# remis-thoughts/native-hdfs-fuse

Measured on AMD Instinct MI355X. Metric: GiB/s CRC32C, device-resident 64 KiB packets × 512 B chunks, 1/2/4/8 GPU, higher is better.
Workload: dtype u32

## Files before the change

### include/hdfs_crc32c_debug.h

```cpp
#ifndef HDFS_CRC32C_DEBUG_H
#define HDFS_CRC32C_DEBUG_H

#include <stddef.h>
#include <stdint.h>

#include "hdfs_crc32c.h"

#ifdef __cplusplus
extern "C" {
#endif


int crc32c_debug_plan(const crc32c_packet *pkts, size_t npkts, void *tiles, size_t tiles_cap, void *gen,
                      size_t gen_cap, uint64_t *ntiles, uint64_t *ngen);
int crc32c_debug_plan_abs(const crc32c_packet *pkts, size_t npkts, int absolute, void *tiles, size_t tiles_cap,
                          void *gen, size_t gen_cap, uint64_t *ntiles, uint64_t *ngen);

int crc32c_debug_write_plan(const crc32c_buffer *buffers, uint32_t n_buffers, uint64_t bufferoffset, uint64_t len,
                            uint64_t blockoffset, uint32_t packetsize, uint32_t bpc, uint64_t counts[6]);

size_t crc32c_debug_lds_image(void *dst, size_t cap, uint32_t *c_lg5, uint32_t *c_small4);

size_t crc32c_debug_lds_image_s4(void *dst, size_t cap, uint32_t flags);
void crc32c_debug_affine_constants(uint32_t flags, uint32_t *c_lg5, uint32_t *c_small4);

int crc32c_debug_blocks_fail_flushes(crc32c_blocks *q, uint32_t n);

int crc32c_debug_blocks_resident_inject(crc32c_blocks *q, int hold, uint32_t fail_waits);

int crc32c_debug_blocks_worker_cpu_ns(crc32c_blocks *q, uint64_t *ns);

uint64_t crc32c_debug_plan_block(const crc32c_plan *plan);

typedef struct crc32c_debug_build {
    uint32_t threads, waves_per_simd, mode, units_per_tile, grid;
} crc32c_debug_build;

int crc32c_debug_select_build(uint32_t ntiles, uint32_t ngen, uint32_t nseg, uint32_t nconst, uint32_t general,
// ... 44 lines not shown
```

### native-hdfs-fuse_amd/__init__.py

```python
from __future__ import annotations

import ctypes
import errno
import numbers
import os
import subprocess

import numpy as np

HERE = os.path.dirname(os.path.abspath(__file__))
LIB_PATH = os.path.join(HERE, "libhdfs_crc32c.so")
DEBUG_LIB_PATH = os.path.join(HERE, "libhdfs_crc32c_debug.so")
INCLUDE_DIR = os.path.join(os.path.dirname(HERE), "include")

CRC32C_BIG_ENDIAN = 0x1
CRC32C_TYPE_CRC32 = 0x2
CRC32C_DEVICE_ADDRESSES = 0x4
CRC32C_CPU_FALLBACK = 0x8
CRC32C_MULTI_SELF_SEND = 0x10
CRC32C_COUNT_COMPLETION = 0x20
CRC32C_MULTI_PIPELINE = 0x40
CRC32C_MULTI_PER_GROUP_RECV = 0x80
CRC32C_VERIFY_OVERLAP = 0x80000000
PATH_NONE, PATH_GPU, PATH_CPU = 0, 1, 2
# ... 165 lines not shown
        "crc32c_plan_exec": (i32, [vp, vp, vp, vp]),
        "crc32c_plan_destroy": (i32, [vp]),
        "crc32c_plan_nchecksums": (u64, [vp]),
        "crc32c_plan_payload_bytes": (u64, [vp]),
        "crc32c_chunks_dev": (i32, [vp, vp, sz, vp, vp, u32, vp]),
        "crc32c_batch_host": (i32, [vp, vp, vp, sz, vp, u32]),
        "crc32c_chunks": (i32, [vp, sz, u32, vp, u32]),
        "crc32c_multi_create": (i32, [vp, i32, pp]),
        "crc32c_multi_destroy": (i32, [vp]),
        "crc32c_multi_batch_host": (i32, [vp, vp, vp, sz, u32, vp, u32]),
        "crc32c_last_error": (ctypes.c_char_p, []),
        "crc32c_debug_plan": (i32, [vp, sz, vp, sz, vp, sz, ctypes.POINTER(u64), ctypes.POINTER(u64)]),
        "crc32c_debug_plan_abs": (i32, [vp, sz, i32, vp, sz, vp, sz, ctypes.POINTER(u64), ctypes.POINTER(u64)]),
        "crc32c_debug_lds_image": (sz, [vp, sz, vp, vp]),
        "crc32c_debug_lds_image_s4": (sz, [vp, sz, u32]),
        "crc32c_plan_verify": (i32, [vp, vp, vp, vp, vp]),
        "crc32c_plan_verify_bitmap": (i32, [vp, vp, vp, vp, vp, vp]),
        "crc32c_frame_packets": (sz, [vp, sz, vp, u32, u64, ctypes.c_int64, u32, vp, sz, vp]),
        "crc32c_block_md5": (None, [vp, sz, u32, vp]),
        "crc32c_md5_nblocks": (u64, [u64, u32]),
        "crc32c_md5_blocks": (i32, [vp, vp, u64, u32, u32, vp, vp]),
        "crc32c_md5_block_list": (i32, [vp, vp, vp, sz, u32, vp, vp]),
        "crc32c_plan_exec_blocks_md5": (i32, [vp, vp, vp, sz, vp, vp]),
        "crc32c_file_md5": (None, [vp, sz, vp]),
        "crc32c_combine": (u32, [u32, u32, u64, u32]),
        "crc32c_block_composite": (i32, [vp, sz, u32, u32, u32, vp]),
        "crc32c_file_composite": (i32, [vp, vp, sz, u32, vp]),
        "crc32c_composite_cells": (i32, [vp, vp, u64, u32, u32, u32, u32, vp, vp]),
        "crc32c_composite_block_list": (i32, [vp, vp, vp, vp, sz, u32, u32, vp, vp]),
        "crc32c_plan_exec_blocks_composite": (i32, [vp, vp, vp, sz, vp, vp]),
# ... 675 lines not shown
    n = int(lib().crc32c_debug_lds_image(None, 0, None, None))
    img = np.zeros(n, np.uint8)
    c_lg = np.zeros(5, np.uint32)
    c_small = np.zeros(4, np.uint32)
    lib().crc32c_debug_lds_image(_np_ptr(img), n, _np_ptr(c_lg), _np_ptr(c_small))
    return img, c_lg, c_small


def debug_lds_image_s4(flags: int = 0):
    n = int(lib().crc32c_debug_lds_image_s4(None, 0, flags))
    img = np.zeros(n, np.uint8)
    lib().crc32c_debug_lds_image_s4(_np_ptr(img), n, flags)
    return img


def debug_affine_constants(flags: int = 0):
    c_lg = np.zeros(5, np.uint32)
    c_small = np.zeros(4, np.uint32)
    lib().crc32c_debug_affine_constants(flags, _np_ptr(c_lg), _np_ptr(c_small))
    return c_lg, c_small
```

### native-hdfs-fuse_amd/csrc/crc32c_device.h

```cpp
#pragma once
#include <hip/hip_runtime.h>
#include <stdint.h>

#include "kernel_abi.h"

namespace hdfs_crc_dev {

using hdfs_crc::ConstRun;
using hdfs_crc::FastTile;
using hdfs_crc::GenItem;
using hdfs_crc::GenPiece;
using hdfs_crc::KParams;
using hdfs_crc::SegItem;
using hdfs_crc::kGeneralTile;
using hdfs_crc::kEpochWord;

constexpr uint32_t kLdsBytes = hdfs_crc::kKernelLdsBytes;
constexpr uint32_t kShiftOff = hdfs_crc::kKernelShiftOff;
constexpr uint32_t kStageBytes = (kLdsBytes + 1023u) / 1024u * 1024u;
static_assert(kStageBytes <= hdfs_crc::kTableAlloc, "staging reads past the device table");
constexpr uint32_t kS4Bytes = uint32_t(hdfs_crc::kS4Bytes);
constexpr uint32_t kS4NibOff = uint32_t(hdfs_crc::kS4NibOff);
constexpr uint32_t kS4ShiftOff = uint32_t(hdfs_crc::kS4ShiftOff);
constexpr uint32_t kS4StageBytes = (kS4Bytes + 1023u) / 1024u * 1024u;
// ... 56 lines not shown
    }
    return acc;
}

__device__ __forceinline__ uint32_t and_or(uint32_t a, uint32_t mask, uint32_t c) {
    uint32_t r;
    asm("v_and_or_b32 %0, %1, %2, %3" : "=v"(r) : "v"(a), "s"(mask), "v"(c));
    return r;
}

struct LaneCols {
    uint32_t col4;
    uint32_t hi;
    uint32_t nib;
    uint32_t toff;
};

constexpr int kImgFull = 0, kImgCompact = 2;
constexpr uint32_t kS4CNibOff = uint32_t(hdfs_crc::kS4CNibOff);
constexpr uint32_t kS4CShiftOff = uint32_t(hdfs_crc::kS4CShiftOff);
constexpr uint32_t kS4CStageBytes = (uint32_t(hdfs_crc::kS4CBytes) + 1023u) / 1024u * 1024u;

template <int IMG>
__device__ __forceinline__ LaneCols lane_cols(uint32_t q) {
    if (IMG == kImgCompact)
        return LaneCols{0u, 2048u, (q << 2) | kS4CNibOff, 1024u};
    return LaneCols{q << 2, (q << 2) | 65536u, (q << 2) | kS4NibOff, 128u};
}

template <int J>
__device__ __forceinline__ uint32_t byte_addr(uint32_t v, uint32_t base) {
    return __builtin_amdgcn_perm(v, base, 0x0C020000u | uint32_t(4 + J) << 8);
}

template <int IMG>
__device__ __forceinline__ uint32_t s4(const uint8_t *lds, const LaneCols &c, uint32_t v, uint32_t next) {
    if (IMG == kImgCompact) {
        const uint32_t a3 = lds_u32(lds, (__builtin_amdgcn_ubfe(v, 0, 8) << 2) + c.hi + c.toff);
        const uint32_t a2 = lds_u32(lds, (__builtin_amdgcn_ubfe(v, 8, 8) << 2) + c.hi);
        const uint32_t a1 = lds_u32(lds, (__builtin_amdgcn_ubfe(v, 16, 8) << 2) + c.toff);
        const uint32_t a0 = lds_u32(lds, (v >> 24) << 2);
        return xor3(xor3(a3, a2, a1), a0, next);
    }
    const uint32_t a3 = lds_u32(lds, byte_addr<0>(v, c.hi) + c.toff);
    const uint32_t a2 = lds_u32(lds, byte_addr<1>(v, c.hi));
    const uint32_t a1 = lds_u32(lds, byte_addr<2>(v, c.col4) + c.toff);
    const uint32_t a0 = lds_u32(lds, byte_addr<3>(v, c.col4));
    return xor3(xor3(a3, a2, a1), a0, next);
}

template <int DIAG, int IMG>
__device__ __forceinline__ uint32_t piece_lin_s4(const uint8_t *lds, uint4 d, const LaneCols &c) {
    if (DIAG == 1) return d.x ^ d.y ^ d.z ^ d.w;
    const uint32_t u = s4<IMG>(lds, c, s4<IMG>(lds, c, s4<IMG>(lds, c, d.x, d.y), d.z), d.w);
    const uint32_t xs[8] = {u << 8, u << 4, u, u >> 4, u >> 8, u >> 12, u >> 16, u >> 20};
    uint32_t r[8];
#pragma unroll
    for (int t = 0; t < 8; ++t) r[t] = lds_u32(lds, and_or(xs[t], 0x0F00u, c.nib) + (t >> 1) * 4096u + (t & 1) * 128u);
    return xor3(xor3(r[0], r[1], r[2]), xor3(r[3], r[4], r[5]), r[6] ^ r[7]);
}

template <bool S4, int DIAG, int IMG>
__device__ __forceinline__ uint32_t piece(const uint8_t *lds, uint4 d, const LaneCols &c) {
    if (S4) return piece_lin_s4<DIAG, IMG>(lds, d, c);
    return piece_lin<DIAG>(lds, d, c.col4);
}

template <bool S4, int IMG>
__device__ __forceinline__ uint32_t zshift(const uint8_t *lds, uint32_t s, uint32_t x) {
    const uint32_t base = (!S4 ? kShiftOff : IMG == kImgCompact ? kS4CShiftOff : kS4ShiftOff) + (s - 1u) * 512u;
    uint32_t r = 0;
#pragma unroll
    for (int t = 0; t < 8; ++t) r ^= lds_u32(lds, base + t * 64u + ((x >> (4 * t)) & 15u) * 4u);
    return r;
}

template <int CTRL>
__device__ __forceinline__ uint32_t dpp(uint32_t v) {
    return static_cast<uint32_t>(__builtin_amdgcn_update_dpp(0, static_cast<int>(v), CTRL, 0xF, 0xF, false));
}
constexpr int kDppXor1 = 0xB1;
constexpr int kDppXor2 = 0x4E;
constexpr int kDppXor8 = 0x128;

template <int XORMASK>
// ... 580 lines not shown

#include "crc32c_items.h"

template <int THREADS, int WPS, int MODE>
__global__ __launch_bounds__(THREADS, WPS) void hdfs_crc32c_plan_kernel(hdfs_crc::KParams p) {
    using namespace hdfs_crc_dev;
    constexpr bool NT = (MODE & kModeNt) != 0;
    constexpr bool S4 = (MODE & kModeS4) != 0;
    constexpr bool STAMPS = (MODE & kModeStamps) != 0;
    constexpr bool COMPDIAG = (MODE & kModeCompDiag) != 0;
    constexpr int DIAG = ((MODE & kModeMemDiag) ? 1 : 0) | ((MODE & kModeGDiagNoGather) ? 2 : 0) |
                         ((MODE & kModeGDiagNoMask) ? 4 : 0);
    constexpr bool NOSTAGE = (MODE & kModeNoStage) != 0;
    constexpr bool VERIFY = (MODE & kModeVerify) != 0;
    constexpr bool C = S4 && (MODE & kModeS4C) != 0;
    constexpr int IMG = C ? kImgCompact : kImgFull;
    constexpr bool GENERAL = (MODE & kModeGeneral) != 0;
    constexpr int GEN = !GENERAL ? 0
                                 : ((MODE & kModeNoGItems) ? 0 : kGenItems) |
                                       ((MODE & kModeNoShift) ? ((MODE & kModeGGroup2) ? kGenGroup2 : kGenGroup4)
                                                              : (kGenShift | kGenGroup2)) |
                                       ((MODE & kModeGHoist) ? kGenHoist : 0) | ((MODE & kModeHalfT) ? kGenHalf : 0) |
                                       ((!(MODE & (kModeNoGItems | kModeNoPadT))) ? kGenPadded : 0);
    constexpr bool EARLY = (MODE & kModeEarly) != 0;
    constexpr bool OVL = !EARLY && (MODE & kModeOvl) != 0;
    constexpr bool QUARTER = (MODE & kModeQuarter) != 0;
    constexpr bool XCDMAP = (MODE & kModeXcdMap) != 0;
    constexpr int SPLIT = (MODE & kModeHalves) ? 2 : 4;
    constexpr int AUX = NT ? 2 : 0;
    constexpr uint32_t kWaves = THREADS / 64;
    constexpr uint32_t kStage = !S4 ? kStageBytes : C ? kS4CStageBytes : kS4StageBytes;
    __shared__ __attribute__((aligned(16))) uint8_t lds[kStage + 32 + (VERIFY ? 4 * kBadList : 0)];
    uint32_t *pool_ctr = reinterpret_cast<uint32_t *>(lds + kStage);
    uint32_t *vacc = pool_ctr + 1;
    uint32_t *exit_ctr = pool_ctr + 5;
    const uint8_t *table = !S4 ? p.table : C ? p.table_s4 + hdfs_crc::kS4COff : p.table_s4;
    const int lane = int(threadIdx.x & 63u);
    const uint32_t wv = __builtin_amdgcn_readfirstlane(threadIdx.x >> 6);

    uint64_t t_start = 0, t_staged = 0;
    if (STAMPS) t_start = __builtin_amdgcn_s_memrealtime();

    const uint64_t nunits = QUARTER ? uint64_t(SPLIT) * p.ntiles : uint64_t(p.ntiles);
    const uint32_t rng = XCDMAP && (gridDim.x % 8u) == 0 ? (blockIdx.x % 8u) * (gridDim.x / 8u) + blockIdx.x / 8u
                                                         : blockIdx.x;
    const uint32_t tbeg = uint32_t((nunits * rng) / gridDim.x);
    const uint32_t tend = uint32_t((nunits * (rng + 1)) / gridDim.x);
    if (threadIdx.x == 0) {
        *pool_ctr = tbeg + kWaves;
        *exit_ctr = 0;
        if (VERIFY) {
// ... 7 lines not shown
    FastTile ft{0, 0, 0};
    uint4 v[9];
    uint32_t ev = 0;
    int kind = 1;
    auto load_next = [&](uint32_t j) {
        if (QUARTER) {
            kind = load_unit<AUX, COMPDIAG, VERIFY, GEN, SPLIT>(p, j, lane, ft, v, ev);
        } else {
            ft = tile_at(p, j);
            load_any<AUX, COMPDIAG, VERIFY, GEN>(p, ft, lane, v, ev);
        }
    };
    if (EARLY && t < tend) load_next(t);
    const bool tables = (p.ntiles | p.ngen | p.nseg) != 0;
    constexpr uint32_t kStageChunks = kStage / 1024u;
    constexpr uint32_t kNoZChunks = !S4 ? kStageChunks : C ? uint32_t(hdfs_crc::kS4CShiftOff / 1024u)
                                                           : uint32_t(hdfs_crc::kS4ShiftOff / 1024u);
    static_assert(!S4 || kNoZChunks * 1024u == (C ? hdfs_crc::kS4CShiftOff : hdfs_crc::kS4ShiftOff),
                  "the Z section starts on a staging chunk");
    const uint32_t nstage = p.skip_z ? kNoZChunks : kStageChunks;
    if (!NOSTAGE && tables) {
        const uint32_t rot = (blockIdx.x * 37u) % nstage;
        for (uint32_t i = wv; i < nstage; i += kWaves) {
            const uint32_t c = i + rot < nstage ? i + rot : i + rot - nstage;
            __builtin_amdgcn_global_load_lds(
                (const __attribute__((address_space(1))) void *)(table + c * 1024u + 16u * uint32_t(lane)),
                (__attribute__((address_space(3))) void *)(lds + c * 1024u), 16, 0, 0);
        }
    }
    if (OVL && t < tend) load_next(t);
    __syncthreads();
    if (STAMPS) t_staged = __builtin_amdgcn_s_memrealtime();
    if (VERIFY && blockIdx.x == 0 && wv == kWaves - 1) verify_init(p, lane);

// ... 55 lines not shown
```

### native-hdfs-fuse_amd/csrc/crc32c_runtime.hip

```cpp
#include <hip/hip_runtime.h>

#include <algorithm>
#include <atomic>
#include <cerrno>
#include <chrono>
#include <cstdarg>
#include <cstdio>
#include <cstdlib>
#include <cstring>
#include <memory>
#include <mutex>
#include <string>
#include <thread>
#include <vector>

#include "crc_math.h"
#include "hdfs_crc32c.h"
#include "hdfs_crc32c_debug.h"
#include "kernel_abi.h"
#include "plan.h"
#include "host_copy.h"
#include "runtime_internal.h"

namespace {
// ... 832 lines not shown
    HIP_TRY(preload_md5_kernels());
    HIP_TRY(preload_composite_kernels());
    c->host_pool.pinned = true;
    HIP_TRY(hipStreamCreateWithFlags(&c->upload_stream, hipStreamNonBlocking));
    for (int ty = 0; ty < 2; ++ty) {
        const uint32_t poly = ty ? kPolyIeee : kPoly;
        std::vector<uint8_t> img(kTableAlloc, 0);
        build_lds_image(img.data(), poly);
        affine_constants(c->c_lg[ty], c->c_small[ty], poly);
        HIP_TRY(hipMalloc(reinterpret_cast<void **>(&c->d_table[ty]), kTableAlloc));
        HIP_TRY(hipMemcpy(c->d_table[ty], img.data(), kTableAlloc, hipMemcpyHostToDevice));
        std::vector<uint8_t> img4(kTableAllocS4Full, 0);
        build_lds_image_s4(img4.data(), poly);
        compact_s4_image(img4.data(), img4.data() + kS4COff);
        zero_crc_table(reinterpret_cast<uint32_t *>(img4.data() + kZeroCrcOff), poly);
        HIP_TRY(hipMalloc(reinterpret_cast<void **>(&c->d_table_s4[ty]), kTableAllocS4Full));
        HIP_TRY(hipMemcpy(c->d_table_s4[ty], img4.data(), kTableAllocS4Full, hipMemcpyHostToDevice));
    }
    *out = c.release();
    return 0;
}

}

namespace {

void ctx_teardown(crc32c_ctx *ctx) {
    {
        DeviceGuard guard(ctx->device);
        for (Stage &s : ctx->stage) free_stage(s);
// ... 360 lines not shown
```

### native-hdfs-fuse_amd/csrc/crc_math.cpp

```cpp
#include "crc_math.h"

#include <cstring>
#include <mutex>
#include <vector>

namespace hdfs_crc {

namespace {
struct PolyTable {
    uint32_t t[256];
    std::once_flag once;
};
PolyTable g_tab[2];

void init_t0(uint32_t poly, uint32_t *t) {
    for (uint32_t b = 0; b < 256; ++b) {
        uint32_t r = b;
        for (int i = 0; i < 8; ++i) r = (r >> 1) ^ (poly & (0u - (r & 1u)));
        t[b] = r;
    }
}
}

const uint32_t *byte_table(uint32_t poly) {
// ... 131 lines not shown
                    zq.apply(s4_step(n << (4 * t), poly)));
    }
    std::vector<uint8_t> nib(kLdsBytes);
    build_lds_image(nib.data(), poly);
    std::memcpy(dst + kS4ShiftOff, nib.data() + kLdsShiftOff, kMaxShift * 512);
}

void compact_s4_image(const uint8_t *full, uint8_t *dst) {
    std::memset(dst, 0, kS4CBytes);
    for (uint32_t m = 0; m < 4; ++m)
        for (uint32_t b = 0; b < 256; ++b)
            std::memcpy(dst + m * 1024u + 4u * b, full + (m >> 1) * 65536u + b * 256u + (m & 1u) * 128u, 4);
    std::memcpy(dst + kS4CNibOff, full + kS4NibOff, kS4Bytes - kS4NibOff);
}

void affine_constants(uint32_t c_lg[5], uint32_t c_small[4], uint32_t poly) {
    for (int lg = 0; lg < 5; ++lg) c_lg[lg] = op_zeros(512ull << lg, poly).apply(0xffffffffu) ^ 0xffffffffu;
    for (int r = 0; r < 4; ++r) c_small[r] = op_zeros(r, poly).apply(0xffffffffu) ^ 0xffffffffu;
}

void zero_crc_table(uint32_t *dst, uint32_t poly) {
    uint32_t reg = 0xffffffffu;
    for (uint32_t n = 0; n <= kZeroCrcMax; ++n) {
        dst[n] = reg ^ 0xffffffffu;
        reg = append_zero_byte(reg, poly);
    }
}

}
```

### native-hdfs-fuse_amd/csrc/crc_math.h

```cpp
#pragma once
#include <cstddef>
#include <cstdint>

namespace hdfs_crc {

constexpr uint32_t kPoly = 0x82f63b78u;
constexpr uint32_t kPolyIeee = 0xedb88320u;

struct Gf2Op {
    uint32_t col[32];
    uint32_t apply(uint32_t v) const {
        uint32_t r = 0;
        for (int j = 0; v; ++j, v >>= 1)
            if (v & 1u) r ^= col[j];
        return r;
    }
};

const uint32_t *byte_table(uint32_t poly = kPoly);
uint32_t append_zero_byte(uint32_t reg, uint32_t poly = kPoly);
Gf2Op op_identity();
Gf2Op op_compose(const Gf2Op &a, const Gf2Op &b);
Gf2Op op_zeros(uint64_t nbytes, uint32_t poly = kPoly);
uint32_t shift_zeros(uint32_t reg, uint64_t nbytes, uint32_t poly = kPoly);
// ... 12 lines not shown
constexpr size_t kLdsShiftOff = 65536;
constexpr int kMaxShift = 15;
constexpr size_t kLdsBytes = kLdsPosBytes + kMaxShift * 512;

void build_lds_image(uint8_t *dst, uint32_t poly = kPoly);

constexpr size_t kS4NibOff = 131072;
constexpr size_t kS4ShiftOff = 147456;
constexpr size_t kS4Bytes = kS4ShiftOff + kMaxShift * 512;

constexpr size_t kS4CNibOff = 4096;
constexpr size_t kS4CShiftOff = kS4CNibOff + (kS4ShiftOff - kS4NibOff);
constexpr size_t kS4CBytes = kS4CShiftOff + kMaxShift * 512;
void compact_s4_image(const uint8_t *full, uint8_t *dst);

void build_lds_image_s4(uint8_t *dst, uint32_t poly = kPoly);
uint32_t s4_step(uint32_t u, uint32_t poly = kPoly);

void affine_constants(uint32_t c_lg[5], uint32_t c_small[4], uint32_t poly = kPoly);

constexpr uint32_t kZeroCrcMax = 8192;
void zero_crc_table(uint32_t *dst, uint32_t poly = kPoly);

}
```

### native-hdfs-fuse_amd/csrc/debug/crc32c_variants.hip

```cpp
#include "../crc32c_device.h"
#include "../runtime_internal.h"
#include "hdfs_crc32c_debug.h"

namespace {

using namespace hdfs_crc_dev;
constexpr int kS4Nt = kModeS4 | kModeNt | kModeGeneral;

struct Variant {
    int id;
    const char *name;
    uint32_t threads, wg_per_cu;
    bool exact;
    bool prod_grid = false;
};

constexpr Variant kVariants[] = {
    {0, "s4_nt", 768, 1, true},
    {1, "nibble_wg1024x2_nt", 1024, 2, true},
    {2, "s4_wg1024x1_nt", 1024, 1, true},
    {3, "s4_wg768x1_nt_memonly", 768, 1, false},
    {4, "s4_wg768x1_nt_compute_only", 768, 1, false},
    {5, "s4_wg768x1_nt_stamps", 768, 1, true},
    {6, "s4_wg768x1_nt_memonly_stamps", 768, 1, false},
// ... 33 lines not shown
    {82, "s4c_nt_quarter_nopad_prodgrid", 768, 1, true, true},
    {83, "s4c_nt_quarter_nopad_early_prodgrid", 768, 1, true, true},
    {84, "s4c_nt_nopad_prodgrid", 768, 1, true, true},
    {85, "s4c_nt_nopad_early_prodgrid", 768, 1, true, true},
    {86, "s4c_nt_halves_nopad_prodgrid", 768, 1, true, true},
    {87, "s4c_wg1024_nt_halves_nopad_prodgrid", 1024, 1, true, true},
    {88, "s4c_wg1024_nt_nopad_prodgrid", 1024, 1, true, true},
    {89, "s4c_nt_pow2only_quarter_early_prodgrid", 768, 1, true, true},
    {90, "s4c_nt_pow2only_quarter_prodgrid", 768, 1, true, true},
    {91, "s4c_nt_pow2only_halves_prodgrid", 768, 1, true, true},
    {92, "s4c_nt_pow2only_prodgrid", 768, 1, true, true},
    {93, "s4c_wg512_nt_pow2only_quarter_early_prodgrid", 512, 1, true, true},
    {94, "s4c_wg512_nt_pow2only_prodgrid", 512, 1, true, true},
    {95, "s4c_wg512_nt_quarter_nopad_early_prodgrid", 512, 1, true, true},
    {96, "s4_nt_nostage_prodgrid", 768, 1, false, true},
};

const Variant *find(int v) {
    for (const Variant &x : kVariants)
        if (x.id == v) return &x;
    return nullptr;
}

#define HDFS_LAUNCH(T, W, M) hipLaunchKernelGGL((hdfs_crc32c_plan_kernel<T, W, M>), g, b, 0, stream, p)

hipError_t launch_variant(const hdfs_crc::KParams &p, const Variant &v, uint32_t num_cu, hipStream_t stream) {
    const uint64_t items = uint64_t(p.ntiles) + (uint64_t(p.ngen) + 1) / 2 + (uint64_t(p.nseg) + 1) / 2 + p.nconst;
    const uint64_t waves = v.threads / 64;
    const uint32_t units = ((v.id >= 51 && v.id <= 55) || v.id == 82 || v.id == 83 || v.id == 89 || v.id == 90 ||
                            v.id == 93 || v.id == 95)
                               ? 4u
                           : (v.id == 60 || v.id == 61 || v.id == 86 || v.id == 87 || v.id == 91)             ? 2u
                                                                                                              : 1u;
    uint64_t grid = v.prod_grid ? hdfs_crc::production_grid(p, num_cu, units) : (items + waves - 1) / waves;
    const uint64_t cap = uint64_t(num_cu) * v.wg_per_cu;
    if (grid > cap) grid = cap;
    if (grid == 0) grid = 1;
    const dim3 g{uint32_t(grid), 1, 1}, b{v.threads, 1, 1};
    if (((v.id >= 82 && v.id <= 88) || v.id == 95) && (p.general & (hdfs_crc::kGeneralPadded | hdfs_crc::kGeneralHalf)))
        return hipErrorInvalidValue;
    if (v.id >= 89 && v.id <= 94 && p.general) return hipErrorInvalidValue;
    switch (v.id) {
    case 1: HDFS_LAUNCH(1024, 8, kModeNt | kModeGeneral); break;
    case 2: HDFS_LAUNCH(1024, 4, kS4Nt); break;
    case 3: HDFS_LAUNCH(768, 3, kS4Nt | kModeMemDiag); break;
    case 4: HDFS_LAUNCH(768, 3, kS4Nt | kModeCompDiag); break;
    case 5: HDFS_LAUNCH(768, 3, kS4Nt | kModeStamps); break;
    case 6: HDFS_LAUNCH(768, 3, kS4Nt | kModeMemDiag | kModeStamps); break;
    case 7: HDFS_LAUNCH(768, 3, kS4Nt | kModeMemDiag | kModeNoStage); break;
    case 9: HDFS_LAUNCH(512, 2, kS4Nt); break;
    case 40: HDFS_LAUNCH(768, 3, kS4Nt | kModeMemDiag | kModeNoStage); break;
    case 41: HDFS_LAUNCH(768, 3, kS4Nt | kModeS4C); break;
    case 42: HDFS_LAUNCH(768, 3, kS4Nt | kModeS4C | kModeStamps); break;
    case 43: HDFS_LAUNCH(768, 3, kS4Nt | kModeStamps); break;
    case 44: HDFS_LAUNCH(256, 4, kS4Nt | kModeS4C); break;
    case 45: HDFS_LAUNCH(128, 4, kS4Nt | kModeS4C); break;
// ... 25 lines not shown
    case 82: HDFS_LAUNCH(768, 3, kS4Nt | kModeS4C | kModeNoPadT | kModeQuarter); break;
    case 83: HDFS_LAUNCH(768, 3, kS4Nt | kModeS4C | kModeNoPadT | kModeQuarter | kModeEarly); break;
    case 84: HDFS_LAUNCH(768, 3, kS4Nt | kModeS4C | kModeNoPadT); break;
    case 85: HDFS_LAUNCH(768, 3, kS4Nt | kModeS4C | kModeNoPadT | kModeEarly); break;
    case 86: HDFS_LAUNCH(768, 3, kS4Nt | kModeS4C | kModeNoPadT | kModeQuarter | kModeHalves); break;
    case 87: HDFS_LAUNCH(1024, 4, kS4Nt | kModeS4C | kModeNoPadT | kModeQuarter | kModeHalves); break;
    case 88: HDFS_LAUNCH(1024, 4, kS4Nt | kModeS4C | kModeNoPadT); break;
    case 89: HDFS_LAUNCH(768, 3, kModeS4 | kModeNt | kModeS4C | kModeQuarter | kModeEarly); break;
    case 90: HDFS_LAUNCH(768, 3, kModeS4 | kModeNt | kModeS4C | kModeQuarter); break;
    case 91: HDFS_LAUNCH(768, 3, kModeS4 | kModeNt | kModeS4C | kModeQuarter | kModeHalves); break;
    case 92: HDFS_LAUNCH(768, 3, kModeS4 | kModeNt | kModeS4C); break;
    case 93: HDFS_LAUNCH(512, 2, kModeS4 | kModeNt | kModeS4C | kModeQuarter | kModeEarly); break;
    case 94: HDFS_LAUNCH(512, 2, kModeS4 | kModeNt | kModeS4C); break;
    case 95: HDFS_LAUNCH(512, 2, kS4Nt | kModeS4C | kModeNoPadT | kModeQuarter | kModeEarly); break;
    case 96: HDFS_LAUNCH(768, 3, kS4Nt | kModeNoStage); break;
    default: return hipErrorInvalidValue;
    }
    return hipGetLastError();
}
#undef HDFS_LAUNCH

}

extern "C" int crc32c_debug_plan_exec_variant(crc32c_plan *plan, const void *dev_payload, uint32_t *dev_out,
                                              uint64_t *dev_stamps, int variant, void *stream) {
    using namespace hdfs_crc;
    if (!plan) return fail(-EINVAL, "plan == NULL");
    const Variant *v = find(variant);
    if (!v) return fail(-EINVAL, "kernel variant %d is not built", variant);
    if (plan->nchecksums == 0) return 0;
// ... 23 lines not shown
```

### native-hdfs-fuse_amd/csrc/kernel_abi.h

```cpp
#pragma once
#include <hip/hip_runtime.h>
#include <stdint.h>

#include "crc_math.h"
#include "plan.h"
#include "plan_select.h"

namespace hdfs_crc {

constexpr uint32_t kKernelLdsBytes = uint32_t(kLdsBytes);
constexpr uint32_t kKernelShiftOff = uint32_t(kLdsShiftOff);
constexpr uint32_t kTableAlloc = ((kKernelLdsBytes + 16384 - 1) / 16384) * 16384;
constexpr uint32_t kTableAllocS4 = ((uint32_t(kS4Bytes) + 16384 - 1) / 16384) * 16384;
constexpr uint32_t kS4COff = kTableAllocS4;
constexpr uint32_t kTableAllocS4C = ((uint32_t(kS4CBytes) + 16384 - 1) / 16384) * 16384;
constexpr uint32_t kZeroCrcOff = kS4COff + kTableAllocS4C;
constexpr uint32_t kTableAllocS4Full = kZeroCrcOff + ((4 * (kZeroCrcMax + 1) + 16384 - 1) / 16384) * 16384;

struct BlockRef {
    uint64_t payload_delta;
    uint32_t out_delta;
    uint32_t reserved;
};
constexpr uint32_t kMaxLaunchBlocks = 32;

struct KParams {
    const FastTile *tiles;
    const GenItem *gen;
    const SegItem *seg;
    const GenPiece *pieces;
    const ConstRun *consts;
    const uint8_t *payload;
// ... 54 lines not shown
```

### native-hdfs-fuse_amd/csrc/plan.cpp

```cpp
#include <cstdlib>
#include "plan.h"
#include "hdfs_crc32c.h"

#include <algorithm>
#include <cerrno>
#include <cstring>

#include "crc_math.h"
#include "hdfs_crc32c_debug.h"

namespace hdfs_crc {

static int fast_lg(uint32_t bpc) {
    for (int lg = 0; lg <= 4; ++lg)
        if (bpc == (kBlockBytes << lg)) return lg;
    return -1;
}

void HostPlan::clear() {
    tiles.clear();
    gen.clear();
    seg.clear();
    pieces.clear();
    consts.clear();
// ... 432 lines not shown
    return 0;
}

extern "C" size_t crc32c_debug_lds_image(void *dst, size_t cap, uint32_t *c_lg, uint32_t *c_small) {
    if (dst && cap >= hdfs_crc::kLdsBytes) hdfs_crc::build_lds_image(static_cast<uint8_t *>(dst));
    if (c_lg && c_small) hdfs_crc::affine_constants(c_lg, c_small);
    return hdfs_crc::kLdsBytes;
}

extern "C" size_t crc32c_debug_lds_image_s4(void *dst, size_t cap, uint32_t flags) {
    const uint32_t poly = (flags & CRC32C_TYPE_CRC32) ? hdfs_crc::kPolyIeee : hdfs_crc::kPoly;
    if (dst && cap >= hdfs_crc::kS4Bytes) hdfs_crc::build_lds_image_s4(static_cast<uint8_t *>(dst), poly);
    return hdfs_crc::kS4Bytes;
}

extern "C" void crc32c_debug_affine_constants(uint32_t flags, uint32_t *c_lg, uint32_t *c_small) {
    const uint32_t poly = (flags & CRC32C_TYPE_CRC32) ? hdfs_crc::kPolyIeee : hdfs_crc::kPoly;
    hdfs_crc::affine_constants(c_lg, c_small, poly);
}
```

### native-hdfs-fuse_amd/csrc/plan_select.h

```cpp
#pragma once
#include <stdint.h>

namespace hdfs_crc_dev {

constexpr int kModeNt = 1;
constexpr int kModeS4 = 2;
constexpr int kModeStamps = 4;
constexpr int kModeMemDiag = 8;
constexpr int kModeCompDiag = 16;
constexpr int kModeNoStage = 32;
constexpr int kModeVerify = 64;
constexpr int kModeS4C = 512;
constexpr int kModeEarly = 1024;
constexpr int kModeHalves = 16384;
constexpr int kModeQuarter = 4096;
constexpr int kModeXcdMap = 2048;
constexpr int kModeGDiagNoGather = 128;
constexpr int kModeGDiagNoMask = 8192;
constexpr int kModeGeneral = 256;
constexpr int kModeNoShift = 32768;
constexpr int kModeNoGItems = 65536;
constexpr int kModeGHoist = 131072;
constexpr int kModeGGroup2 = 262144;
constexpr int kModeHalfT = 1048576;
constexpr int kModeNoPadT = 2097152;
constexpr int kModeOvl = 524288;

}

namespace hdfs_crc {

constexpr uint32_t kGeneralItems = 1u, kGeneralShift = 2u, kGeneralHalf = 4u, kGeneralPadded = 8u;

constexpr uint64_t kSmallBatchItemsPerCu = 16;
constexpr uint64_t kQuarterTilesPerCu = 3;
constexpr uint64_t kEarlyTilesPerCu = 2;
constexpr uint64_t kHalvesTilesPerCu = 6;

inline uint64_t launch_items(uint32_t ntiles, uint32_t ngen, uint32_t nseg, uint32_t nconst,
                             uint32_t units_per_tile = 1) {
    return uint64_t(ntiles) * units_per_tile + (uint64_t(ngen) + 1) / 2 + (uint64_t(nseg) + 1) / 2 + nconst;
// ... 58 lines not shown
```

### native-hdfs-fuse_amd/csrc/resident_engine.h

```cpp
#pragma once
#include <hip/hip_runtime.h>

#include <cstdint>

#include "crc32c_device.h"
#include "hdfs_crc32c.h"
#include "runtime_internal.h"

namespace hdfs_crc_res {

using namespace hdfs_crc_dev;
using hdfs_crc::FastTile;

constexpr uint32_t kRing = 64;
constexpr uint32_t kMaxWg = 256;
constexpr uint64_t kTicksPerUs = 100;
constexpr uint64_t kStuckMs = 50;
constexpr uint32_t kStampRing = 4096;
constexpr uint64_t kWorkerMs = 200;

constexpr int kTagShift = 48;
constexpr uint64_t kAddrMask = (1ull << kTagShift) - 1;
constexpr uint64_t kTagMask = 0x7fffull << kTagShift;
constexpr uint64_t kShapeFlag = 1ull << 63;
// ... 81 lines not shown
        v[i] = make_uint4(r[0], r[1], r[2], r[3]);
    }
}
__device__ __forceinline__ void rstore(uint32_t *out, uint32_t idx, uint32_t v) {
    typedef __attribute__((address_space(1))) uint32_t *GU32;
    __hip_atomic_store((GU32)(out + idx), v, __ATOMIC_RELAXED, __HIP_MEMORY_SCOPE_SYSTEM);
}
__device__ __forceinline__ void rtile_reduce(const RParams &p, const uint8_t *lds, uint32_t *out, const FastTile &t,
                                             const uint32_t pc[8], int lane) {
    const uint32_t nb = t.meta & 0xffu, lg = (t.meta >> 8) & 0xffu;
    uint32_t x = block_lin(pc, lane);
    const uint32_t blk = rep_block(lane);
    if (lg) {
        const uint32_t nbc = 1u << lg;
        const uint32_t s = nbc - 1u - (blk & (nbc - 1u));
        if (s) x = zshift<true, kImgFull>(lds, s, x);
        x ^= static_cast<uint32_t>(__shfl_xor(static_cast<int>(x), 32));
        if (lg >= 2) x ^= dpp<kDppXor8>(x);
        if (lg >= 3) x ^= dpp<kDppXor2>(x);
        if (lg >= 4) x ^= dpp<kDppXor1>(x);
    }
    if (rep_lane(lane, blk, nb, lg)) rstore(out, t.out + (blk >> lg), out_order(x ^ p.c_lg[lg], p.flags));
}
__device__ __forceinline__ void rtile_finish(const RParams &p, const uint8_t *lds, uint32_t *out, const FastTile &t,
                                             uint4 v[8], int lane) {
    uint32_t pc[8];
    tile_pieces<0, true, kImgFull>(lds, v, pc, lane, NoPrep{});
    rtile_reduce(p, lds, out, t, pc, lane);
}
__device__ __forceinline__ void run_tile(const RParams &p, const uint8_t *lds, const uint8_t *payload,
                                         uint32_t *out, const FastTile *tiles, uint32_t idx, int lane) {
    const FastTile t = rtile(tiles, idx);
    uint4 v[8];
    rtile_load(payload, t, lane, v);
    __builtin_amdgcn_sched_barrier(0);
    rtile_finish(p, lds, out, t, v, lane);
}
__device__ __forceinline__ void run_tile_pair(const RParams &p, const uint8_t *lds, const uint8_t *payload,
                                              uint32_t *out, const FastTile *tiles, uint32_t ia, uint32_t ib,
                                              int lane) {
    const FastTile ta = rtile(tiles, ia), tb = rtile(tiles, ib);
    uint4 va[8], vb[8];
// ... 9 lines not shown
    const uint32_t r = uint32_t(reinterpret_cast<uintptr_t>(payload + t.src)) & 15u;
    if (!r) {
        uint4 v[8];
        rtile_load(payload, t, lane, v);
        __builtin_amdgcn_sched_barrier(0);
        rtile_finish(p, lds, out, t, v, lane);
        return;
    }
    uint4 v[9];
    load_shifted_raw<2>(payload, t, r, lane, v);
    __builtin_amdgcn_sched_barrier(0);
    uint32_t pc[8];
    const uint32_t b = r & 3u, li = ((t.meta & 0xffu) - 1u) >> 1;
    const int ll = int(((t.meta & 0xffu) - 1u) & 1u) * 32 + 31;
    switch (r >> 2) {
        case 0: tile_pieces<0, true, kImgFull>(lds, v, pc, lane, ShiftPrep<0>{v, b, lane, li, ll}); break;
        case 1: tile_pieces<0, true, kImgFull>(lds, v, pc, lane, ShiftPrep<1>{v, b, lane, li, ll}); break;
        case 2: tile_pieces<0, true, kImgFull>(lds, v, pc, lane, ShiftPrep<2>{v, b, lane, li, ll}); break;
        default: tile_pieces<0, true, kImgFull>(lds, v, pc, lane, ShiftPrep<3>{v, b, lane, li, ll}); break;
    }
    rtile_reduce(p, lds, out, t, pc, lane);
}

__device__ __forceinline__ void run_gen_item(const RParams &p, const uint8_t *lds, const uint8_t *payload,
                                             uint32_t *out, const GenItem &g, bool valid, int lane) {
    const uint32_t acc = gen_item_lin<true, kImgFull>(payload, lds, g, lane);
    if (valid && (lane & 31) == 0)
        rstore(out, g.out, out_order(acc ^ (g.len >= 4 ? 0xffffffffu : p.c_small[g.len]), p.flags));
}

__device__ __forceinline__ void run_gtile(const RParams &p, const uint8_t *lds, const uint8_t *payload, uint32_t *out,
                                          const FastTile &t, int lane) {
    const GShape g = gshape(t);
    const uint32_t lg = 31u - uint32_t(__builtin_clz(g.k));
    for (uint32_t s = 0; 16u * s < g.nfb; ++s) {
        const uint32_t nb = min(g.nfb - 16u * s, 16u);
        run_ptile(p, lds, payload, out, FastTile{g.src + 8192u * s, t.out + ((16u * s) >> lg), nb | (lg << 8)}, lane);
    }
    if (g.tl) {
        const GenItem gi{g.src + uint64_t(g.nch) * g.bpc, t.out + g.nch, g.tl};
        const bool valid = (lane >> 5) == 0;
// ... 142 lines not shown
        if (stop && col >= fwd) break;
        if (stop && now() - last > kStuckMs * 1000 * kTicksPerUs) break;
        if (now() - last > kWorkerMs * 1000 * kTicksPerUs) break;
        __builtin_amdgcn_s_sleep(1);
    }
    if (lane == 0) {
        st_sys(&h->exit_col, col);
        wait_vmem();
        st_sys(&h->exits, ld_sys(&h->exits) + 1);
    }
}

template <uint32_t kWaves, uint32_t kPhases, uint32_t kPer, bool GENERAL = false>
__global__ __launch_bounds__(kWaves * 64, kWaves / 4) void resident_kernel(RParams p) {
    constexpr uint32_t kWorkers = kWaves - 1;
    constexpr uint32_t kStage = kS4StageBytes;
    __shared__ __attribute__((aligned(16))) uint8_t lds[kStage + 4 * kRing];
    uint32_t *lcnt = reinterpret_cast<uint32_t *>(lds + kStage);
    const int lane = int(threadIdx.x & 63u);
    const uint32_t wv = __builtin_amdgcn_readfirstlane(threadIdx.x >> 6);
    constexpr uint32_t kChunks = kStage / 1024u;
    const uint32_t rot = (blockIdx.x * 37u) % kChunks;
    for (uint32_t i = wv; i < kChunks; i += kWaves) {
        const uint32_t c = i + rot < kChunks ? i + rot : i + rot - kChunks;
        __builtin_amdgcn_global_load_lds(
            (const __attribute__((address_space(1))) void *)(p.table_s4 + c * 1024u + 16u * uint32_t(lane)),
            (__attribute__((address_space(3))) void *)(lds + c * 1024u), 16, 0, 0);
    }
    if (threadIdx.x < kRing) lcnt[threadIdx.x] = 0;
    __syncthreads();
    if (wv == kWaves - 1) {
        if (blockIdx.x == 0) forwarder<GENERAL>(p, lane);
        if (blockIdx.x == 1) collector(p, lane);
        return;
    }
    const uint32_t b = blockIdx.x, G = gridDim.x;
    const uint32_t phase = (b + wv) % kPhases;
    uint32_t rank = 0, expect = 0;
    for (uint32_t w = 0; w < kWorkers; ++w)
        if ((b + w) % kPhases == phase) {
            if (w < wv) ++rank;
// ... 61 lines not shown
```

Baseline: 5831.

## Add split S4 LDS table image and make it the default S4 layout

Adds a new S4 table layout that interleaves the four byte-slice tables per byte value into 256-byte rows within a 64 KiB region, so each lookup address comes from one v_perm of the input word against a per-lane column. The main and resident kernels now stage and index this split image by default (with a lean variant that derives selectors by XOR), shrinking the staged LDS footprint and the address arithmetic per lookup. The device table allocation grows to hold the extra image, and the old layout stays reachable through a new Img32 mode flag. Risks include changed LDS bank-conflict patterns and correctness of the selector encoding.

```diff
diff --git a/include/hdfs_crc32c_debug.h b/include/hdfs_crc32c_debug.h
--- a/include/hdfs_crc32c_debug.h
+++ b/include/hdfs_crc32c_debug.h
@@ -22,6 +22,7 @@
 size_t crc32c_debug_lds_image(void *dst, size_t cap, uint32_t *c_lg5, uint32_t *c_small4);
 
 size_t crc32c_debug_lds_image_s4(void *dst, size_t cap, uint32_t flags);
+size_t crc32c_debug_lds_image_s4_split(void *dst, size_t cap, uint32_t flags);
 void crc32c_debug_affine_constants(uint32_t flags, uint32_t *c_lg5, uint32_t *c_small4);
 
 int crc32c_debug_blocks_fail_flushes(crc32c_blocks *q, uint32_t n);
diff --git a/native-hdfs-fuse_amd/__init__.py b/native-hdfs-fuse_amd/__init__.py
--- a/native-hdfs-fuse_amd/__init__.py
+++ b/native-hdfs-fuse_amd/__init__.py
@@ -203,6 +203,7 @@
         "crc32c_debug_plan_abs": (i32, [vp, sz, i32, vp, sz, vp, sz, ctypes.POINTER(u64), ctypes.POINTER(u64)]),
         "crc32c_debug_lds_image": (sz, [vp, sz, vp, vp]),
         "crc32c_debug_lds_image_s4": (sz, [vp, sz, u32]),
+        "crc32c_debug_lds_image_s4_split": (sz, [vp, sz, u32]),
         "crc32c_plan_verify": (i32, [vp, vp, vp, vp, vp]),
         "crc32c_plan_verify_bitmap": (i32, [vp, vp, vp, vp, vp, vp]),
         "crc32c_frame_packets": (sz, [vp, sz, vp, u32, u64, ctypes.c_int64, u32, vp, sz, vp]),
@@ -908,6 +909,13 @@
     return img
 
 
+def debug_lds_image_s4_split(flags: int = 0):
+    n = int(lib().crc32c_debug_lds_image_s4_split(None, 0, flags))
+    img = np.zeros(n, np.uint8)
+    lib().crc32c_debug_lds_image_s4_split(_np_ptr(img), n, flags)
+    return img
+
+
 def debug_affine_constants(flags: int = 0):
     c_lg = np.zeros(5, np.uint32)
     c_small = np.zeros(4, np.uint32)
diff --git a/native-hdfs-fuse_amd/csrc/crc32c_device.h b/native-hdfs-fuse_amd/csrc/crc32c_device.h
--- a/native-hdfs-fuse_amd/csrc/crc32c_device.h
+++ b/native-hdfs-fuse_amd/csrc/crc32c_device.h
@@ -94,23 +94,49 @@
     uint32_t hi;
     uint32_t nib;
     uint32_t toff;
+    uint32_t sel[4];
 };
 
-constexpr int kImgFull = 0, kImgCompact = 2;
+constexpr int kImgFull = 0, kImgSplit = 1, kImgCompact = 2, kImgSplitLean = 3;
+constexpr bool is_split(int img) { return img == kImgSplit || img == kImgSplitLean; }
 constexpr uint32_t kS4CNibOff = uint32_t(hdfs_crc::kS4CNibOff);
 constexpr uint32_t kS4CShiftOff = uint32_t(hdfs_crc::kS4CShiftOff);
 constexpr uint32_t kS4CStageBytes = (uint32_t(hdfs_crc::kS4CBytes) + 1023u) / 1024u * 1024u;
+constexpr uint32_t kS4SNibOff = uint32_t(hdfs_crc::kS4SNibOff);
+constexpr uint32_t kS4SShiftOff = uint32_t(hdfs_crc::kS4SShiftOff);
+constexpr uint32_t kS4SStageBytes = (uint32_t(hdfs_crc::kS4SBytes) + 1023u) / 1024u * 1024u;
+static_assert(kS4SStageBytes <= hdfs_crc::kTableAllocS4S, "staging reads past the device table");
+
+template <int IMG>
+struct S4Image {
+    static constexpr uint32_t kStage = IMG == kImgCompact ? kS4CStageBytes : is_split(IMG) ? kS4SStageBytes : kS4StageBytes;
+    static constexpr uint32_t kShift = IMG == kImgCompact ? kS4CShiftOff : is_split(IMG) ? kS4SShiftOff : kS4ShiftOff;
+    static constexpr uint32_t kTableOff = IMG == kImgCompact ? hdfs_crc::kS4COff : is_split(IMG) ? hdfs_crc::kS4SOff : 0u;
+};
 
 template <int IMG>
 __device__ __forceinline__ LaneCols lane_cols(uint32_t q) {
     if (IMG == kImgCompact)
-        return LaneCols{0u, 2048u, (q << 2) | kS4CNibOff, 1024u};
-    return LaneCols{q << 2, (q << 2) | 65536u, (q << 2) | kS4NibOff, 128u};
+        return LaneCols{0u, 2048u, (q << 2) | kS4CNibOff, 1024u, {0u, 0u, 0u, 0u}};
+    if (is_split(IMG)) {
+        const uint32_t col4 = q << 2;
+        const uint32_t a = q < 16u ? 0x0C0C0700u : 0x0C0C0600u;
+        return LaneCols{col4 | (col4 ^ 64u) << 8, 0u, col4 | kS4SNibOff, 64u,
+                        {a, a ^ 0x0101u, a ^ 0x0200u, a ^ 0x0301u}};
+    }
+    return LaneCols{q << 2, (q << 2) | 65536u, (q << 2) | kS4NibOff, 128u, {0u, 0u, 0u, 0u}};
 }
 
 template <int J>
 __device__ __forceinline__ uint32_t byte_addr(uint32_t v, uint32_t base) {
     return __builtin_amdgcn_perm(v, base, 0x0C020000u | uint32_t(4 + J) << 8);
+}
+
+template <uint32_t K>
+__device__ __forceinline__ uint32_t sel_xor(uint32_t sel, uint32_t at) {
+    uint32_t r;
+    asm("v_xor_b32 %0, %1, %2 ; %3" : "=v"(r) : "n"(K), "v"(sel), "v"(at));
+    return r;
 }
 
 template <int IMG>
@@ -122,6 +148,17 @@
         const uint32_t a0 = lds_u32(lds, (v >> 24) << 2);
         return xor3(xor3(a3, a2, a1), a0, next);
     }
+    if (is_split(IMG)) {
+        const bool lean = IMG == kImgSplitLean;
+        const uint32_t s1 = lean ? sel_xor<0x0101u>(c.sel[0], v) : c.sel[1];
+        const uint32_t s2 = lean ? sel_xor<0x0200u>(c.sel[0], v) : c.sel[2];
+        const uint32_t s3 = lean ? sel_xor<0x0301u>(c.sel[0], v) : c.sel[3];
+        const uint32_t a = lds_u32(lds, __builtin_amdgcn_perm(v, c.col4, c.sel[0]));
+        const uint32_t b = lds_u32(lds, __builtin_amdgcn_perm(v, c.col4, s1));
+        const uint32_t cc = lds_u32(lds, __builtin_amdgcn_perm(v, c.col4, s2) + 128u);
+        const uint32_t d = lds_u32(lds, __builtin_amdgcn_perm(v, c.col4, s3) + 128u);
+        return xor3(xor3(cc, d, a), b, next);
+    }
     const uint32_t a3 = lds_u32(lds, byte_addr<0>(v, c.hi) + c.toff);
     const uint32_t a2 = lds_u32(lds, byte_addr<1>(v, c.hi));
     const uint32_t a1 = lds_u32(lds, byte_addr<2>(v, c.col4) + c.toff);
@@ -148,7 +185,7 @@
 
 template <bool S4, int IMG>
 __device__ __forceinline__ uint32_t zshift(const uint8_t *lds, uint32_t s, uint32_t x) {
-    const uint32_t base = (!S4 ? kShiftOff : IMG == kImgCompact ? kS4CShiftOff : kS4ShiftOff) + (s - 1u) * 512u;
+    const uint32_t base = (!S4 ? kShiftOff : S4Image<IMG>::kShift) + (s - 1u) * 512u;
     uint32_t r = 0;
 #pragma unroll
     for (int t = 0; t < 8; ++t) r ^= lds_u32(lds, base + t * 64u + ((x >> (4 * t)) & 15u) * 4u);
@@ -759,7 +796,6 @@
     constexpr bool NOSTAGE = (MODE & kModeNoStage) != 0;
     constexpr bool VERIFY = (MODE & kModeVerify) != 0;
     constexpr bool C = S4 && (MODE & kModeS4C) != 0;
-    constexpr int IMG = C ? kImgCompact : kImgFull;
     constexpr bool GENERAL = (MODE & kModeGeneral) != 0;
     constexpr int GEN = !GENERAL ? 0
                                  : ((MODE & kModeNoGItems) ? 0 : kGenItems) |
@@ -767,6 +803,8 @@
                                                               : (kGenShift | kGenGroup2)) |
                                        ((MODE & kModeGHoist) ? kGenHoist : 0) | ((MODE & kModeHalfT) ? kGenHalf : 0) |
                                        ((!(MODE & (kModeNoGItems | kModeNoPadT))) ? kGenPadded : 0);
+    constexpr bool LEAN = (GEN & kGenItems) && (GEN & (kGenShift | kGenHalf));
+    constexpr int IMG = C ? kImgCompact : (!S4 || (MODE & kModeImg32)) ? kImgFull : LEAN ? kImgSplitLean : kImgSplit;
     constexpr bool EARLY = (MODE & kModeEarly) != 0;
     constexpr bool OVL = !EARLY && (MODE & kModeOvl) != 0;
     constexpr bool QUARTER = (MODE & kModeQuarter) != 0;
@@ -774,12 +812,12 @@
     constexpr int SPLIT = (MODE & kModeHalves) ? 2 : 4;
     constexpr int AUX = NT ? 2 : 0;
     constexpr uint32_t kWaves = THREADS / 64;
-    constexpr uint32_t kStage = !S4 ? kStageBytes : C ? kS4CStageBytes : kS4StageBytes;
+    constexpr uint32_t kStage = !S4 ? kStageBytes : S4Image<IMG>::kStage;
     __shared__ __attribute__((aligned(16))) uint8_t lds[kStage + 32 + (VERIFY ? 4 * kBadList : 0)];
     uint32_t *pool_ctr = reinterpret_cast<uint32_t *>(lds + kStage);
     uint32_t *vacc = pool_ctr + 1;
     uint32_t *exit_ctr = pool_ctr + 5;
-    const uint8_t *table = !S4 ? p.table : C ? p.table_s4 + hdfs_crc::kS4COff : p.table_s4;
+    const uint8_t *table = !S4 ? p.table : p.table_s4 + S4Image<IMG>::kTableOff;
     const int lane = int(threadIdx.x & 63u);
     const uint32_t wv = __builtin_amdgcn_readfirstlane(threadIdx.x >> 6);
 
@@ -817,10 +855,8 @@
     if (EARLY && t < tend) load_next(t);
     const bool tables = (p.ntiles | p.ngen | p.nseg) != 0;
     constexpr uint32_t kStageChunks = kStage / 1024u;
-    constexpr uint32_t kNoZChunks = !S4 ? kStageChunks : C ? uint32_t(hdfs_crc::kS4CShiftOff / 1024u)
-                                                           : uint32_t(hdfs_crc::kS4ShiftOff / 1024u);
-    static_assert(!S4 || kNoZChunks * 1024u == (C ? hdfs_crc::kS4CShiftOff : hdfs_crc::kS4ShiftOff),
-                  "the Z section starts on a staging chunk");
+    constexpr uint32_t kNoZChunks = !S4 ? kStageChunks : S4Image<IMG>::kShift / 1024u;
+    static_assert(!S4 || kNoZChunks * 1024u == S4Image<IMG>::kShift, "the Z section starts on a staging chunk");
     const uint32_t nstage = p.skip_z ? kNoZChunks : kStageChunks;
     if (!NOSTAGE && tables) {
         const uint32_t rot = (blockIdx.x * 37u) % nstage;
diff --git a/native-hdfs-fuse_amd/csrc/crc32c_runtime.hip b/native-hdfs-fuse_amd/csrc/crc32c_runtime.hip
--- a/native-hdfs-fuse_amd/csrc/crc32c_runtime.hip
+++ b/native-hdfs-fuse_amd/csrc/crc32c_runtime.hip
@@ -870,6 +870,7 @@
         build_lds_image_s4(img4.data(), poly);
         compact_s4_image(img4.data(), img4.data() + kS4COff);
         zero_crc_table(reinterpret_cast<uint32_t *>(img4.data() + kZeroCrcOff), poly);
+        split_s4_image(img4.data(), img4.data() + kS4SOff);
         HIP_TRY(hipMalloc(reinterpret_cast<void **>(&c->d_table_s4[ty]), kTableAllocS4Full));
         HIP_TRY(hipMemcpy(c->d_table_s4[ty], img4.data(), kTableAllocS4Full, hipMemcpyHostToDevice));
     }
diff --git a/native-hdfs-fuse_amd/csrc/crc_math.cpp b/native-hdfs-fuse_amd/csrc/crc_math.cpp
--- a/native-hdfs-fuse_amd/csrc/crc_math.cpp
+++ b/native-hdfs-fuse_amd/csrc/crc_math.cpp
@@ -169,6 +169,13 @@
     std::memcpy(dst + kS4CNibOff, full + kS4NibOff, kS4Bytes - kS4NibOff);
 }
 
+void split_s4_image(const uint8_t *full, uint8_t *dst) {
+    for (uint32_t b = 0; b < 256; ++b)
+        for (uint32_t m = 0; m < 4; ++m)
+            std::memcpy(dst + b * 256u + m * 64u, full + (m >> 1) * 65536u + b * 256u + (m & 1u) * 128u, 64);
+    std::memcpy(dst + kS4SNibOff, full + kS4NibOff, kS4Bytes - kS4NibOff);
+}
+
 void affine_constants(uint32_t c_lg[5], uint32_t c_small[4], uint32_t poly) {
     for (int lg = 0; lg < 5; ++lg) c_lg[lg] = op_zeros(512ull << lg, poly).apply(0xffffffffu) ^ 0xffffffffu;
     for (int r = 0; r < 4; ++r) c_small[r] = op_zeros(r, poly).apply(0xffffffffu) ^ 0xffffffffu;
diff --git a/native-hdfs-fuse_amd/csrc/crc_math.h b/native-hdfs-fuse_amd/csrc/crc_math.h
--- a/native-hdfs-fuse_amd/csrc/crc_math.h
+++ b/native-hdfs-fuse_amd/csrc/crc_math.h
@@ -50,6 +50,11 @@
 constexpr size_t kS4CBytes = kS4CShiftOff + kMaxShift * 512;
 void compact_s4_image(const uint8_t *full, uint8_t *dst);
 
+constexpr size_t kS4SNibOff = 65536;
+constexpr size_t kS4SShiftOff = kS4SNibOff + (kS4ShiftOff - kS4NibOff);
+constexpr size_t kS4SBytes = kS4SShiftOff + kMaxShift * 512;
+void split_s4_image(const uint8_t *full, uint8_t *dst);
+
 void build_lds_image_s4(uint8_t *dst, uint32_t poly = kPoly);
 uint32_t s4_step(uint32_t u, uint32_t poly = kPoly);
 
diff --git a/native-hdfs-fuse_amd/csrc/debug/crc32c_variants.hip b/native-hdfs-fuse_amd/csrc/debug/crc32c_variants.hip
--- a/native-hdfs-fuse_amd/csrc/debug/crc32c_variants.hip
+++ b/native-hdfs-fuse_amd/csrc/debug/crc32c_variants.hip
@@ -71,6 +71,9 @@
     {94, "s4c_wg512_nt_pow2only_prodgrid", 512, 1, true, true},
     {95, "s4c_wg512_nt_quarter_nopad_early_prodgrid", 512, 1, true, true},
     {96, "s4_nt_nostage_prodgrid", 768, 1, false, true},
+    {97, "s4_nt_pow2only_img32_prodgrid", 768, 1, true, true},
+    {98, "s4_nt_pow2only_img32_stamps_prodgrid", 768, 1, true, true},
+    {99, "s4_nt_pow2only_stamps_prodgrid", 768, 1, true, true},
 };
 
 const Variant *find(int v) {
@@ -96,7 +99,7 @@
     const dim3 g{uint32_t(grid), 1, 1}, b{v.threads, 1, 1};
     if (((v.id >= 82 && v.id <= 88) || v.id == 95) && (p.general & (hdfs_crc::kGeneralPadded | hdfs_crc::kGeneralHalf)))
         return hipErrorInvalidValue;
-    if (v.id >= 89 && v.id <= 94 && p.general) return hipErrorInvalidValue;
+    if (((v.id >= 89 && v.id <= 94) || (v.id >= 97 && v.id <= 99)) && p.general) return hipErrorInvalidValue;
     switch (v.id) {
     case 1: HDFS_LAUNCH(1024, 8, kModeNt | kModeGeneral); break;
     case 2: HDFS_LAUNCH(1024, 4, kS4Nt); break;
@@ -152,6 +155,9 @@
     case 94: HDFS_LAUNCH(512, 2, kModeS4 | kModeNt | kModeS4C); break;
     case 95: HDFS_LAUNCH(512, 2, kS4Nt | kModeS4C | kModeNoPadT | kModeQuarter | kModeEarly); break;
     case 96: HDFS_LAUNCH(768, 3, kS4Nt | kModeNoStage); break;
+    case 97: HDFS_LAUNCH(768, 3, kModeS4 | kModeNt | kModeImg32); break;
+    case 98: HDFS_LAUNCH(768, 3, kModeS4 | kModeNt | kModeImg32 | kModeStamps); break;
+    case 99: HDFS_LAUNCH(768, 3, kModeS4 | kModeNt | kModeStamps); break;
     default: return hipErrorInvalidValue;
     }
     return hipGetLastError();
diff --git a/native-hdfs-fuse_amd/csrc/kernel_abi.h b/native-hdfs-fuse_amd/csrc/kernel_abi.h
--- a/native-hdfs-fuse_amd/csrc/kernel_abi.h
+++ b/native-hdfs-fuse_amd/csrc/kernel_abi.h
@@ -15,7 +15,9 @@
 constexpr uint32_t kS4COff = kTableAllocS4;
 constexpr uint32_t kTableAllocS4C = ((uint32_t(kS4CBytes) + 16384 - 1) / 16384) * 16384;
 constexpr uint32_t kZeroCrcOff = kS4COff + kTableAllocS4C;
-constexpr uint32_t kTableAllocS4Full = kZeroCrcOff + ((4 * (kZeroCrcMax + 1) + 16384 - 1) / 16384) * 16384;
+constexpr uint32_t kS4SOff = kZeroCrcOff + ((4 * (kZeroCrcMax + 1) + 16384 - 1) / 16384) * 16384;
+constexpr uint32_t kTableAllocS4S = ((uint32_t(kS4SBytes) + 16384 - 1) / 16384) * 16384;
+constexpr uint32_t kTableAllocS4Full = kS4SOff + kTableAllocS4S;
 
 struct BlockRef {
     uint64_t payload_delta;
diff --git a/native-hdfs-fuse_amd/csrc/plan.cpp b/native-hdfs-fuse_amd/csrc/plan.cpp
--- a/native-hdfs-fuse_amd/csrc/plan.cpp
+++ b/native-hdfs-fuse_amd/csrc/plan.cpp
@@ -470,6 +470,16 @@
     return hdfs_crc::kS4Bytes;
 }
 
+extern "C" size_t crc32c_debug_lds_image_s4_split(void *dst, size_t cap, uint32_t flags) {
+    const uint32_t poly = (flags & CRC32C_TYPE_CRC32) ? hdfs_crc::kPolyIeee : hdfs_crc::kPoly;
+    if (dst && cap >= hdfs_crc::kS4SBytes) {
+        std::vector<uint8_t> full(hdfs_crc::kS4Bytes);
+        hdfs_crc::build_lds_image_s4(full.data(), poly);
+        hdfs_crc::split_s4_image(full.data(), static_cast<uint8_t *>(dst));
+    }
+    return hdfs_crc::kS4SBytes;
+}
+
 extern "C" void crc32c_debug_affine_constants(uint32_t flags, uint32_t *c_lg, uint32_t *c_small) {
     const uint32_t poly = (flags & CRC32C_TYPE_CRC32) ? hdfs_crc::kPolyIeee : hdfs_crc::kPoly;
     hdfs_crc::affine_constants(c_lg, c_small, poly);
diff --git a/native-hdfs-fuse_amd/csrc/plan_select.h b/native-hdfs-fuse_amd/csrc/plan_select.h
--- a/native-hdfs-fuse_amd/csrc/plan_select.h
+++ b/native-hdfs-fuse_amd/csrc/plan_select.h
@@ -25,6 +25,7 @@
 constexpr int kModeHalfT = 1048576;
 constexpr int kModeNoPadT = 2097152;
 constexpr int kModeOvl = 524288;
+constexpr int kModeImg32 = 4194304;
 
 }
 
diff --git a/native-hdfs-fuse_amd/csrc/resident_engine.h b/native-hdfs-fuse_amd/csrc/resident_engine.h
--- a/native-hdfs-fuse_amd/csrc/resident_engine.h
+++ b/native-hdfs-fuse_amd/csrc/resident_engine.h
@@ -119,7 +119,7 @@
     if (lg) {
         const uint32_t nbc = 1u << lg;
         const uint32_t s = nbc - 1u - (blk & (nbc - 1u));
-        if (s) x = zshift<true, kImgFull>(lds, s, x);
+        if (s) x = zshift<true, kImgSplit>(lds, s, x);
         x ^= static_cast<uint32_t>(__shfl_xor(static_cast<int>(x), 32));
         if (lg >= 2) x ^= dpp<kDppXor8>(x);
         if (lg >= 3) x ^= dpp<kDppXor2>(x);
@@ -130,7 +130,7 @@
 __device__ __forceinline__ void rtile_finish(const RParams &p, const uint8_t *lds, uint32_t *out, const FastTile &t,
                                              uint4 v[8], int lane) {
     uint32_t pc[8];
-    tile_pieces<0, true, kImgFull>(lds, v, pc, lane, NoPrep{});
+    tile_pieces<0, true, kImgSplit>(lds, v, pc, lane, NoPrep{});
     rtile_reduce(p, lds, out, t, pc, lane);
 }
 __device__ __forceinline__ void run_tile(const RParams &p, const uint8_t *lds, const uint8_t *payload,
@@ -170,17 +170,17 @@
     const uint32_t b = r & 3u, li = ((t.meta & 0xffu) - 1u) >> 1;
     const int ll = int(((t.meta & 0xffu) - 1u) & 1u) * 32 + 31;
     switch (r >> 2) {
-        case 0: tile_pieces<0, true, kImgFull>(lds, v, pc, lane, ShiftPrep<0>{v, b, lane, li, ll}); break;
-        case 1: tile_pieces<0, true, kImgFull>(lds, v, pc, lane, ShiftPrep<1>{v, b, lane, li, ll}); break;
-        case 2: tile_pieces<0, true, kImgFull>(lds, v, pc, lane, ShiftPrep<2>{v, b, lane, li, ll}); break;
-        default: tile_pieces<0, true, kImgFull>(lds, v, pc, lane, ShiftPrep<3>{v, b, lane, li, ll}); break;
+        case 0: tile_pieces<0, true, kImgSplit>(lds, v, pc, lane, ShiftPrep<0>{v, b, lane, li, ll}); break;
+        case 1: tile_pieces<0, true, kImgSplit>(lds, v, pc, lane, ShiftPrep<1>{v, b, lane, li, ll}); break;
+        case 2: tile_pieces<0, true, kImgSplit>(lds, v, pc, lane, ShiftPrep<2>{v, b, lane, li, ll}); break;
+        default: tile_pieces<0, true, kImgSplit>(lds, v, pc, lane, ShiftPrep<3>{v, b, lane, li, ll}); break;
     }
     rtile_reduce(p, lds, out, t, pc, lane);
 }
 
 __device__ __forceinline__ void run_gen_item(const RParams &p, const uint8_t *lds, const uint8_t *payload,
                                              uint32_t *out, const GenItem &g, bool valid, int lane) {
-    const uint32_t acc = gen_item_lin<true, kImgFull>(payload, lds, g, lane);
+    const uint32_t acc = gen_item_lin<true, kImgSplit>(payload, lds, g, lane);
     if (valid && (lane & 31) == 0)
         rstore(out, g.out, out_order(acc ^ (g.len >= 4 ? 0xffffffffu : p.c_small[g.len]), p.flags));
 }
@@ -353,7 +353,7 @@
 template <uint32_t kWaves, uint32_t kPhases, uint32_t kPer, bool GENERAL = false>
 __global__ __launch_bounds__(kWaves * 64, kWaves / 4) void resident_kernel(RParams p) {
     constexpr uint32_t kWorkers = kWaves - 1;
-    constexpr uint32_t kStage = kS4StageBytes;
+    constexpr uint32_t kStage = kS4SStageBytes;
     __shared__ __attribute__((aligned(16))) uint8_t lds[kStage + 4 * kRing];
     uint32_t *lcnt = reinterpret_cast<uint32_t *>(lds + kStage);
     const int lane = int(threadIdx.x & 63u);
@@ -363,7 +363,7 @@
     for (uint32_t i = wv; i < kChunks; i += kWaves) {
         const uint32_t c = i + rot < kChunks ? i + rot : i + rot - kChunks;
         __builtin_amdgcn_global_load_lds(
-            (const __attribute__((address_space(1))) void *)(p.table_s4 + c * 1024u + 16u * uint32_t(lane)),
+            (const __attribute__((address_space(1))) void *)(p.table_s4 + hdfs_crc::kS4SOff + c * 1024u + 16u * uint32_t(lane)),
             (__attribute__((address_space(3))) void *)(lds + c * 1024u), 16, 0, 0);
     }
     if (threadIdx.x < kRing) lcnt[threadIdx.x] = 0;
```

New measurement: 5894 (median of 6 runs). +1.1%, better.
